# zhengxwen/HIBAG

Measured on AMD Instinct MI355X. Metric: hlaPredict() samples/sec, 10k samples x 100-classifier HLA-B, higher is better.
Workload: dtype f64

## Files before the change

hibag_amd/csrc/hibag_device.h:

```cpp
#ifndef HIBAG_DEVICE_H_
#define HIBAG_DEVICE_H_

#include <stdint.h>
#include <hip/hip_vector_types.h>

#define HIBAG_WAVE 64
#define HIBAG_TAB_N 257
#ifndef HIBAG_TILE
#define HIBAG_TILE 15
#endif
#ifndef HIBAG_CHUNK
#define HIBAG_CHUNK 4
#endif
#ifndef HIBAG_BLOCK_WAVES
#define HIBAG_BLOCK_WAVES 4
#endif
#ifndef HIBAG_ACCUM_WAVES
#define HIBAG_ACCUM_WAVES 4
#endif
#define HIBAG_TILE_META (4 + HIBAG_TILE)
static_assert(HIBAG_TILE <= 16, "cell rows are packed 4 bits each");
#define HIBAG_MAX_NWP 12

#define HIBAG_CHUNK_DWORDS(nwp) (HIBAG_CHUNK * ((nwp) + 2))
#define HIBAG_PLIST_DWORDS 32
#define HIBAG_PLIST_END 0x80000000u
#define HIBAG_PLIST_STORE 0x40000000u
#ifndef HIBAG_STORED_PER_VISIT
#define HIBAG_STORED_PER_VISIT 7
#endif
#define HIBAG_ENGINE_VALU 0
#define HIBAG_ENGINE_FP4 1
#define HIBAG_ENGINE_I8 2
#define HIBAG_ENGINE_I8S 3
#define HIBAG_FP4_STEP_SNPS 28
#define HIBAG_FP4_MAX_STEPS 4
#define HIBAG_FP4_STEPS(k) (((k) + HIBAG_FP4_STEP_SNPS - 1) / HIBAG_FP4_STEP_SNPS)
#define HIBAG_FP4_MAX_SNPS 30
#define HIBAG_ENGINE_OF(k, fp4) ((fp4) && (k) <= HIBAG_FP4_MAX_SNPS ? HIBAG_ENGINE_FP4 : (k) < 32 ? HIBAG_ENGINE_I8 : (k) == 32 ? HIBAG_ENGINE_I8S : \
	(fp4) && (k) <= HIBAG_FP4_STEP_SNPS * HIBAG_FP4_MAX_STEPS ? HIBAG_ENGINE_FP4 : HIBAG_ENGINE_VALU)
#define HIBAG_ENGINE_STEPS(e, k) ((e) == HIBAG_ENGINE_FP4 ? (k) <= HIBAG_FP4_MAX_SNPS ? 1 : HIBAG_FP4_STEPS(k) : 1)
#define HIBAG_ENGINE_ROWS(e, k) ((e) == HIBAG_ENGINE_FP4 ? 2 * HIBAG_ENGINE_STEPS(e, k) : ((e) == HIBAG_ENGINE_VALU ? 0 : 4))
#define HIBAG_ENGINE_HAP_DWORDS(e) 12
#define HIBAG_FP4_ENTRY_DWORDS(steps) (8 + 4 * ((steps) - 1))
#define HIBAG_FP4_SCALE_A 54
#define HIBAG_FP4_SCALE_B_LO 54
#define HIBAG_FP4_SCALE_B_HI 55

struct HibagModelView {
	int n_hla;
	int n_classifier;
	int n_snp;
	int n_cell;
	int mask_rows;
	int n_tile;

	const int *n_snp_c;
	const int *nwp;
	const int *snp_off;
	const int *snp_index;
	const int *snp_weight;
	const int *mask_row;
	const int *c_order;
	const int *tile_p0;
	const int *tile_n;
	const uint32_t *tile_meta;
	const uint32_t *cls_cnt;
	const uint32_t *cls_cell;
	const int *cls_off;
	const int *cls_n;
	int n_item, n_split;
	int all_fp4;
	const int *item;
	int n_item_whole, n_item_split;
	const int *item_whole, *item_split;
	double split_heavy_ns, split_rest_ns;
	const int *split_row;
	const int *split_cls;
	const uint64_t *stream_off;
	const uint32_t *stream;
	const double *tab;

	const int *engine;
	const int *n_step;
	int n_valu;
	int n_wide;
	const int *wide_cls;
	int n_wide_scan;
	const int *wide_scan;
	int n_wide_seg;
	const int *wide_seg;
	const uint64_t *wide_seg_off;
	const int *bt_row;
	const uint32_t *hap;
	const uint32_t *hap_off;
	uint32_t hap_dwords;
	const uint64_t *blk_off;
	const int *cls_nblk;
	const uint32_t *plist;
	uint64_t plist_dwords;
	const double *pfac;
	const uint32_t *phdr;
	const uint4 *parow;
	uint64_t parow_blocks;
	int p1_prebuilt;
	const uint32_t *ctile;

	int store_cells;
	const int *cell_row;
	const uint32_t *blk_close;
// ... 37 lines not shown
```

hibag_amd/csrc/hibag_k_pass2.h:

```cpp
#ifndef HIBAG_K_PASS2_H_
#define HIBAG_K_PASS2_H_

typedef uint32_t u32x8 __attribute__((ext_vector_type(8)));

#ifndef ACCUM_OCC
#define ACCUM_OCC 5
#endif

struct AccumAhead {
	u32x8 hv;
	FactorGroup<ACCUM_G>::type F;
	f64x2 winv;
};

__global__ __launch_bounds__(ACCUM_WAVES * HIBAG_WAVE, ACCUM_OCC) void k_accum(HibagModelView M, HibagBatchView B, int n_whole, int K)
{
	__shared__ double tab_s[ACCUM_TAB_N];
	__shared__ double acc_s[ACCUM_WAVES][HIBAG_TILE][HIBAG_WAVE];
#ifdef HIBAG_ACCUM_STAMPS
	__shared__ unsigned long long stamp_s[ACCUM_STAMP_N];
	if (threadIdx.x < ACCUM_STAMP_N) stamp_s[threadIdx.x] = 0;
	unsigned long long stamp_t = 0;
#endif

	const int n_group = B.n_pad / HIBAG_WAVE;
	const int n_gq = ((n_group + 7) / 8 + ACCUM_WAVES - 1) / ACCUM_WAVES;
	const int C = M.n_classifier;
	const int n_item_x = n_gq * M.n_tile;
	const int xcd = blockIdx.x & 7, wx = blockIdx.x >> 3;
	const int wave = __builtin_amdgcn_readfirstlane(threadIdx.x >> 6);
	const int lane = threadIdx.x & 63;
	double (*acc)[HIBAG_WAVE] = acc_s[wave];

	int item = wx, cb = 0, ce = C;
	if (wx >= n_whole) {
		const int rest = n_item_x - n_whole, k = (wx - n_whole) / rest;
		item = n_whole + (wx - n_whole) - k * rest;
		const uint32_t *__restrict__ cum = M.etile_cstart + (size_t)(item % M.n_tile) * (C + 1);
		const uint64_t total = cum[C];
		if (k > 0) cb = chunk_bound(cum, C, (total * (uint64_t)k + K - 1) / K);
		if (k < K - 1) ce = chunk_bound(cum, C, (total * (uint64_t)(k + 1) + K - 1) / K);
		if (cb >= ce) return;
	}
	stage_table(M, tab_s, ACCUM_TAB_N);
	const int jq = item / M.n_tile, tile = item - jq * M.n_tile;
	const int group = (jq * ACCUM_WAVES + wave) * 8 + xcd;
	unsigned long long *flag = B.sync + (size_t)xcd * n_item_x + item;
	if (cb > 0) handover_wait(flag, B, (uint32_t)cb);
#ifdef HIBAG_ACCUM_STAMPS
	int bb_diag = 0, be_diag = 0;
#endif
	if (group < n_group) {
	const int s = group * HIBAG_WAVE + lane;
	const int ncell = M.tile_n[tile];
	const int p0 = M.tile_p0[tile];

	if (cb > 0) {
		double v[HIBAG_TILE];
#pragma unroll
		for (int j = 0; j < HIBAG_TILE; j++) v[j] = load_parked(&B.part[(size_t)(p0 + (j < ncell ? j : 0)) * B.n_pad + s]);
#pragma unroll
		for (int j = 0; j < HIBAG_TILE; j++) acc[j][lane] = v[j];
	} else {
#pragma unroll
		for (int j = 0; j < HIBAG_TILE; j++) acc[j][lane] = 0;
	}

	const ConstPtr<uint32_t> cst = as_const(M.etile_cstart) + (size_t)tile * (C + 1);
	const int bb = __builtin_amdgcn_readfirstlane((int)cst[cb]), be = __builtin_amdgcn_readfirstlane((int)cst[ce]);
#ifdef HIBAG_ACCUM_STAMPS
	if (wave == 0) { bb_diag = bb; be_diag = be; }
#endif
	if (bb < be && !(ABL2_NOLOOP && B.n_pad >= 0)) {
		const uint64_t blk0 = as_const(M.etile_blk0)[tile] + (uint64_t)bb;
		auto bytes32 = [](size_t n) { return n > 0xFFFFFFF0ull ? (int)0xFFFFFFF0u : (int)(uint32_t)n; };
		auto rsrc_flags = [] { int f = 0x00020000; asm volatile("" : "+s"(f)); return f; };
		const __amdgpu_buffer_rsrc_t pr = __builtin_amdgcn_make_buffer_rsrc((void *)(M.parow + blk0 * 64), 0,
			bytes32((size_t)(M.parow_blocks - blk0) * 1024u), rsrc_flags());
		ConstPtr<double> fac = as_const(M.pfac) + blk0 * HIBAG_PLIST_DWORDS;
		ConstPtr<u32x8> eh = (ConstPtr<u32x8>)(as_const(M.ehdr) + blk0 * 8);
		typedef FactorGroup<ACCUM_G>::type AFG;
		const size_t g_bytes = (size_t)group * HIBAG_WAVE * 16u;
		const __amdgpu_buffer_rsrc_t r_bt = __builtin_amdgcn_make_buffer_rsrc((void *)((const char *)B.bt + g_bytes), 0,
			bytes32((size_t)B.bt_rows * B.n_pad * 16u - g_bytes), rsrc_flags());
		const __amdgpu_buffer_rsrc_t r_wi = __builtin_amdgcn_make_buffer_rsrc((void *)((const char *)B.winv + g_bytes), 0,
			bytes32((size_t)C * B.n_pad * 16u - g_bytes), rsrc_flags());
		const __amdgpu_buffer_rsrc_t r_sv = __builtin_amdgcn_make_buffer_rsrc(
			(void *)(B.cells + (size_t)group * (size_t)as_const(M.cell_row)[C] * HIBAG_WAVE), 0,
			bytes32((size_t)as_const(M.cell_row)[C] * HIBAG_WAVE * 8u), rsrc_flags());
		const int vo_a = lane * 16, vo_row = vo_a, vo_sv = lane * 8;
		const uint32_t row_stride = (uint32_t)B.n_pad * 16u;
		constexpr int NS = HIBAG_STORED_PER_VISIT;

		v4i arow, t0, t1;
		double sv[NS];
		double cell = 0;
		auto request_sv = [&](uint32_t w1) {
			const int ns = abl2_stored(w1);
			if (ns > 0) {
				const int sr = (int)(abl2_stored_row(w1) * (uint32_t)(HIBAG_WAVE * 8));
				int vo = vo_sv;
				asm volatile("" : "+v"(vo));
#pragma unroll
				for (int i = 0; i < NS; i++) {
					if (i >= ns) break;
#ifdef HIBAG_ABL2_SVNOLOAD
					asm volatile("" : "=v"(sv[i]));
#elif defined(HIBAG_ABL2_SVX4)
					sv[i] = __builtin_bit_cast(f64x2, __builtin_amdgcn_raw_buffer_load_b128(r_sv, vo + i * HIBAG_WAVE * 8, sr, 2))[0];
#elif defined(HIBAG_ABL2_SVHALF)
					if (i & 1) asm volatile("" : "=v"(sv[i]));
					else sv[i] = __builtin_bit_cast(double, __builtin_amdgcn_raw_buffer_load_b64(r_sv, vo + i * HIBAG_WAVE * 8, sr, 2));
#else
#ifdef HIBAG_SV_PLAIN
					sv[i] = __builtin_bit_cast(double, __builtin_amdgcn_raw_buffer_load_b64(r_sv, vo + i * HIBAG_WAVE * 8, sr, 0));
#else
					sv[i] = __builtin_bit_cast(double, __builtin_amdgcn_raw_buffer_load_b64(r_sv, vo + i * HIBAG_WAVE * 8, sr, 2));
#endif
#endif
				}
			}
		};
		auto request_lane = [&](uint32_t w0, uint32_t w1, int soff_a, f64x2 &winv) {
			arow = __builtin_bit_cast(v4i, __builtin_amdgcn_raw_buffer_load_b128(pr, vo_a, soff_a, 0));
			const int sb = (int)((w0 >> 16) * row_stride);
			t0 = __builtin_bit_cast(v4i, __builtin_amdgcn_raw_buffer_load_b128(r_bt, vo_row, sb, 0));
			t1 = __builtin_bit_cast(v4i, __builtin_amdgcn_raw_buffer_load_b128(r_bt, vo_row, sb + (int)row_stride, 0));
			if (ABL2_NOWINV) winv = f64x2{1.0 + (double)w0, 2.0};
			else winv = __builtin_bit_cast(f64x2, __builtin_amdgcn_raw_buffer_load_b128(r_wi, vo_row, (int)((w0 & 0xFFFFu) * row_stride), 0));
			request_sv(w1);
		};
		auto one_block = [&](const int rel, AccumAhead &cur, AccumAhead &nxt) {
#if defined(HIBAG_ACCUM_PRIO) && HIBAG_ACCUM_PRIO == 1
			__builtin_amdgcn_s_setprio(1);
#elif defined(HIBAG_ACCUM_PRIO) && HIBAG_ACCUM_PRIO == 2
			__builtin_amdgcn_s_setprio(0);
#endif
			const double w_c = cur.winv[0];
			const bool active = w_c > 0;
			const int any = __builtin_popcountll(__ballot(active));
			const double inv_e = cur.winv[1];
			const uint32_t endmask = cur.hv[0];
			const uint32_t gword = cur.hv[6];
			auto live4 = [&](int g) { return g == 0 || gword >= ((uint32_t)(g + 1) << 28); };
			__builtin_amdgcn_sched_barrier(0);
			nxt.hv = eh[rel + 1];
			nxt.F = *(ConstPtr<AFG>)(fac + (size_t)(rel + 1) * HIBAG_PLIST_DWORDS);
			typedef const volatile __attribute__((address_space(4))) uint32_t *TouchPtr;
			const TouchPtr touch = (TouchPtr)(uintptr_t)(fac + (size_t)(rel + 1) * HIBAG_PLIST_DWORDS);
			const uint32_t tch0 = touch[16], tch1 = touch[32], tch2 = touch[48];
			ACCUM_STAMP(0);
			int eval = ABL2_NOEVAL ? 0 : (any != 0 ? (int)(gword >> 28) : 0), eval_b = eval;
			asm volatile("" : "+s"(eval), "+s"(eval_b));
			{
				const int ns = abl2_stored(cur.hv[1]);
				if (!any) asm volatile("v_mov_b64 %0, 0" : "+v"(cell));
				else {
					asm volatile("");
					if (ns > 0) {
						uint32_t jps = cur.hv[6];
#pragma unroll
						for (int i = 0; i < NS; i++) {
							if (i >= ns) break;
#ifdef HIBAG_ABL2_SVNOADD
							asm volatile("" :: "v"(sv[i]));
#else
							__hip_atomic_fetch_add(&acc[(int)(jps & 15)][lane], (sv[i] * inv_e) * w_c, __ATOMIC_RELAXED, __HIP_MEMORY_SCOPE_WORKGROUP);
#endif
							jps >>= 4;
						}
					}
				}
			}
			__builtin_amdgcn_sched_barrier(0);
			ACCUM_STAMP(1);
			v16i D0, D1;
			if (eval) {
				v16f d0, d1;
#pragma unroll
				for (int r = 0; r < 16; r++) { d0[r] = 0.0f; d1[r] = 0.0f; }
				const v8i a8 = {arow[0], arow[1], arow[2], arow[3], 0, 0, 0, 0};
				const v8i b0 = {t0[0], t0[1], t0[2], t0[3], 0, 0, 0, 0};
				const v8i b1 = {t1[0], t1[1], t1[2], t1[3], 0, 0, 0, 0};
				const int sbs = lane >= 32 ? HIBAG_FP4_SCALE_B_HI : HIBAG_FP4_SCALE_B_LO;
				d0 = __builtin_amdgcn_mfma_scale_f32_32x32x64_f8f6f4(a8, b0, d0, 4, 4, 0, HIBAG_FP4_SCALE_A, 0, sbs);
				d1 = __builtin_amdgcn_mfma_scale_f32_32x32x64_f8f6f4(a8, b1, d1, 4, 4, 0, HIBAG_FP4_SCALE_A, 0, sbs);
				D0 = __builtin_bit_cast(v16i, d0);
				D1 = __builtin_bit_cast(v16i, d1);
			}
			__builtin_amdgcn_sched_barrier(0);
			ACCUM_STAMP(2);
			request_lane(cur.hv[2], cur.hv[3], (rel + 1) * 1024, nxt.winv);
			__builtin_amdgcn_sched_barrier(0);
			ACCUM_STAMP(3);
#if defined(HIBAG_ACCUM_PRIO) && HIBAG_ACCUM_PRIO == 1
			__builtin_amdgcn_s_setprio(0);
#elif defined(HIBAG_ACCUM_PRIO) && HIBAG_ACCUM_PRIO == 2
			__builtin_amdgcn_s_setprio(1);
#endif
			if (eval_b) {
				block_own_sample(D0, D1, [&](int g) { return live4(2 * g); });
#ifdef HIBAG_ACCUM_STAMPS
				asm volatile("" :: "v"(D0[0]), "v"(D1[0]));
				ACCUM_STAMP(4);
#endif
				const uint32_t jp_lo = cur.hv[4], jp_hi = cur.hv[5];
				auto fin = [&](double c, bool, int slot) {
					uint32_t row;
					asm volatile("s_bfe_u32 %0, %1, %2" : "=s"(row) : "s"(slot < 16 ? jp_lo : jp_hi), "n"(4 * ((slot >> 1) & 7) | (4 << 16)) : "scc");
					const double v = (c * inv_e) * w_c;
#ifdef HIBAG_ABL2_NOADD
					asm volatile("" :: "v"(v), "s"(row));
#else
					__hip_atomic_fetch_add(&acc[(int)row][lane], v, __ATOMIC_RELAXED, __HIP_MEMORY_SCOPE_WORKGROUP);
#endif
				};
				uint32_t fresh = (cur.hv[1] >> 29) & 1u;
				block_accumulate<ACCUM_G, ACCUM_AHEAD>(fac + (size_t)rel * HIBAG_PLIST_DWORDS, cur.F, endmask, 0u, live4, D0, D1, cell, fresh, tab_s, fin);
			}
			asm volatile("" :: "s"(tch0), "s"(tch1), "s"(tch2), "s"(nxt.hv[7]));
			ACCUM_STAMP(5);
		};

		AccumAhead A, Bn;
		A.hv = eh[0];
		A.F = *(ConstPtr<AFG>)fac;
		request_lane(A.hv[7], A.hv[1], 0, A.winv);
#ifdef HIBAG_ACCUM_STAMPS
		stamp_t = __builtin_readcyclecounter();
#endif
		const int nb = be - bb;
		for (int rel = 0;;) {
			one_block(rel, A, Bn);
			if (++rel >= nb) break;
			one_block(rel, Bn, A);
			if (++rel >= nb) break;
		}
	}

	if (ce < C) for (int j = 0; j < ncell; j++) store_parked(&B.part[(size_t)(p0 + j) * B.n_pad + s], acc[j][lane]);
	else for (int j = 0; j < ncell; j++) B.part[(size_t)(p0 + j) * B.n_pad + s] = acc[j][lane];
	if (tile == 0 && ce == C) ensemble_scalars<8>(M, B, s, nullptr);
	}
#ifdef HIBAG_ACCUM_STAMPS
	__syncthreads();
	if (threadIdx.x < ACCUM_STAMP_N)
		atomicAdd(reinterpret_cast<unsigned long long *>(B.err_dev + 4) + 2000 + threadIdx.x, stamp_s[threadIdx.x]);
	if (threadIdx.x == ACCUM_STAMP_N) atomicAdd(reinterpret_cast<unsigned long long *>(B.err_dev + 4) + 2000 + ACCUM_STAMP_N, (unsigned long long)(be_diag - bb_diag) * ACCUM_WAVES);
#endif
	if (ce < C) handover_post(flag, B.epoch, (uint32_t)ce, B.drop_post == 2 && blockIdx.x == 8 * n_whole);
}

#define CELLS_WAVES 4
#ifndef CELLS_OCC
#define CELLS_OCC 4
#endif
__global__ __launch_bounds__(CELLS_WAVES * HIBAG_WAVE, CELLS_OCC) void k_accum_cells(HibagModelView M, HibagBatchView B)
{
	constexpr int CELLS_V = (HIBAG_TILE + 3) / 4 * 4;
	__shared__ double acc_s[CELLS_WAVES][HIBAG_TILE][HIBAG_WAVE];
	const int n_group = B.n_pad / HIBAG_WAVE;
	const int tq = (M.n_tile + CELLS_WAVES - 1) / CELLS_WAVES;
	const int xcd = blockIdx.x & 7, jb = blockIdx.x >> 3;
	const int wave = __builtin_amdgcn_readfirstlane(threadIdx.x >> 6);
	const int lane = threadIdx.x & 63;
	const int group = (jb / tq) * 8 + xcd, tile = (jb % tq) * CELLS_WAVES + wave;
	if (group >= n_group || tile >= M.n_tile) return;
	const int s = group * HIBAG_WAVE + lane;
	const int C = M.n_classifier;
	const int ncell = M.tile_n[tile];
	double (*acc)[HIBAG_WAVE] = acc_s[wave];
#pragma unroll
	for (int q = 0; q < HIBAG_TILE; q++) acc[q][lane] = 0;

	typedef uint32_t u32x8 __attribute__((ext_vector_type(8)));
	const ConstPtr<u32x8> ct = as_const(reinterpret_cast<const u32x8 *>(M.ctile)) + tile;
	const double *__restrict__ const group_rows = B.cells + (size_t)group * (size_t)as_const(M.cell_row)[C] * HIBAG_WAVE + lane;
	struct Visit { u32x8 rec; double w, inv; };
	auto visit = [&](int c) {
		Visit x;
		x.rec = ct[(size_t)c * M.n_tile];
		x.w = B.cw[(size_t)c * B.n_pad + s];
		x.inv = B.inv[(size_t)c * B.n_pad + s];
		return x;
	};
	auto fetch = [&](const Visit &x, double (&v)[CELLS_V]) {
		const int n = (int)((x.rec[0] >> 8) & 31u);
		const double *__restrict__ rows = group_rows + (size_t)(x.rec[5] & 0x7FFFFFFu) * HIBAG_WAVE;
#pragma unroll
		for (int g = 0; g < HIBAG_TILE; g += 4) {
			if (g >= n) break;
#pragma unroll
			for (int i = g; i < g + 4; i++) v[i] = __builtin_nontemporal_load(rows + (size_t)(i < n ? i : n - 1) * HIBAG_WAVE);
		}
	};
	auto add = [&](int c, const Visit &x, const double (&v)[CELLS_V]) {
		const bool active = x.w > 0;
		if (__ballot(active) == 0) return;
// ... 37 lines not shown
```

hibag_amd/csrc/hibag_model.hip:

```cpp

#include "hibag_internal.h"

namespace hibag_detail {



void build_table(double *tab)
{
	const double min_rare_freq = 1e-5;
	for (int i = 0; i < HIBAG_TAB_N; i++) tab[i] = std::exp(i * std::log(min_rare_freq));
	tab[0] = 1;
	for (int i = 0; i < HIBAG_TAB_N; i++)
		if (!std::isfinite(tab[i])) tab[i] = 0;
}

int check_classifier_args(hibag_hip_model *m, int n_snp_c, const int32_t *snpidx, int n_haplo,
	const double *freq, const int32_t *hla)
{
	if (!m) return hibag_fail(HIBAG_HIP_EINVAL, "model is NULL");
	if (m->finalized) return hibag_fail(HIBAG_HIP_ESTATE, "model already finalized");
	if (n_snp_c < 0 || n_snp_c > HIBAG_HIP_MAX_SNP_IN_CLASSIFIER)
		return hibag_fail(HIBAG_HIP_EINVAL, "there are too many SNP markers in a classifier (%d > %d).",
			n_snp_c, HIBAG_HIP_MAX_SNP_IN_CLASSIFIER);
	if (n_haplo < 0 || (n_haplo > 0 && (!freq || !hla)))
// ... 369 lines not shown
			}
			me[0] = (uint32_t)k;
			me[2] = (uint32_t)jpack; me[3] = (uint32_t)(jpack >> 32);
			{
				uint64_t jp = 0;
				int nl = 0, ns = 0;
				for (int j = 0; j < tile_n[t]; j++)
					if (cell_chunks[c][tile_p0[t] + j] && !stored_big(c, tile_p0[t] + j)) {
						jp |= (uint64_t)j << (4 * nl++);
						if (store_mode != 1) m->second_pass_pairs += pass2_evaluates(c) ? cell_pairs[c][tile_p0[t] + j] : 0;
					}
				for (int j = 0; j < tile_n[t]; j++)
					if (stored_big(c, tile_p0[t] + j)) jp |= (uint64_t)j << (4 * (nl + ns++));
				tile_jpack[(size_t)c * n_tile + t] = jp;
				tile_nlist[(size_t)c * n_tile + t] = (uint32_t)nl;
				tile_nstored[(size_t)c * n_tile + t] = (uint32_t)ns;
				if (store_mode == 2) tile_k0[(size_t)c * n_tile + t] = (uint32_t)n_stored_c[c];
				n_stored_c[c] += ns;
			}
			k_first += k;
			for (int j = 0; j < tile_n[t]; j++)
				if (!cell_chunks[c][tile_p0[t] + j]) me[4 + k++] = (uint32_t)j << 24;
		}
	}
	if (cls_cnt.empty()) { cls_cnt.push_back(0); cls_cell.push_back(0); }

	std::vector<int> item, item_whole, split_row(std::max(C, 1), -1), split_cls, wide_cls;
	double split_heavy_ns = 0, split_rest_ns = 0;
	{
		std::vector<double> work(C, 0.0);
		double typical = 0;
		int n_typ = 0;
		for (int c = 0; c < C; c++) {
			work[c] = (double)pairs[c] * (mfma_nkb[c] ? 50.0 * (0.5 + 0.5 * n_step[c]) : 48.0 * nwp[c]);
			if (mfma_nkb[c]) { typical += work[c]; n_typ++; }
			split_rest_ns += work[c];
		}
		typical = n_typ ? typical / n_typ : 0;
		std::vector<std::pair<double, std::vector<int>>> items, whole;
		for (int c = 0; c < C; c++) {
			if (n_step[c] > 1) { wide_cls.push_back(c); continue; }
			whole.push_back({work[c], {c, 0, cls_n[c], 0}});
			int nseg = 1;
			if (!mfma_nkb[c] && typical > 0 && work[c] > 3 * typical)
				nseg = (int)std::min<double>(64, std::max(2.0, std::floor(work[c] / typical)));
			if (nseg == 1 || cls_n[c] < 2) {
				items.push_back({work[c], {c, 0, cls_n[c], 0}});
				continue;
			}
			split_heavy_ns = std::max(split_heavy_ns, (double)pairs[c] * 18.0 * nwp[c]);
			split_row[c] = 1;
			split_cls.push_back(c);
			uint64_t total = 0, acc = 0, chunk0 = 0;
			for (int i = 0; i < cls_n[c]; i++) total += cls_cnt[cls_off[c] + i] + 1;
			int i0 = 0, k = 1;
			for (int i = 0; i < cls_n[c]; i++) {
				acc += cls_cnt[cls_off[c] + i] + 1;
				const bool last = i + 1 == cls_n[c];
				if (last || acc * nseg >= total * k) {
					uint64_t chunks = 0;
					for (int j = i0; j <= i; j++) chunks += cls_cnt[cls_off[c] + j];
					items.push_back({work[c] * (double)(chunks + 1) / (double)total, {c, i0, i + 1, (int)chunk0}});
					chunk0 += chunks;
					i0 = i + 1;
					while (k < nseg && acc * nseg >= total * k) k++;
				}
			}
		}
		std::stable_sort(whole.begin(), whole.end(), [](const auto &a, const auto &b) { return a.first > b.first; });
		for (const auto &it : whole) item_whole.insert(item_whole.end(), it.second.begin(), it.second.end());
		std::stable_sort(items.begin(), items.end(), [](const auto &a, const auto &b) { return a.first > b.first; });
		for (const auto &it : items) item.insert(item.end(), it.second.begin(), it.second.end());
	}

	std::vector<uint32_t> plist;
	struct SlotRange { size_t first, n; int c; };
	std::vector<SlotRange> slot_ranges;
	std::vector<uint64_t> blk_off(std::max(C, 1), 0), seg_off((size_t)std::max(C, 1) * n_tile, 0);
	std::vector<uint32_t> seg_nblk((size_t)std::max(C, 1) * n_tile, 0);
	long long dbg_b1 = 0, dbg_b2 = 0, dbg_seg = 0;
	std::vector<int> cell_row((size_t)C + 1, 0);
	for (int c = 0; c < C; c++)
		cell_row[c + 1] = cell_row[c] + (store_mode == 1 || split_row[c] >= 0 ? cls_n[c] : store_mode == 2 ? n_stored_c[c] : 0);
	std::vector<uint32_t> ehdr, etile_cstart((size_t)n_tile * (C + 1), 0);
	std::vector<uint64_t> etile_blk0(std::max(n_tile, 1), 0);
	hap.insert(hap.end(), HIBAG_ENGINE_HAP_DWORDS(HIBAG_ENGINE_FP4), 0u);
	while (hap.size() % 4) hap.push_back(0u);
	for (int t = 0; t < n_tile && store_mode != 1; t++) {
		etile_blk0[t] = plist.size() / HIBAG_PLIST_DWORDS;
		for (int c = 0; c < C; c++) {
			const size_t ct = (size_t)c * n_tile + t;
			etile_cstart[(size_t)t * (C + 1) + c] = (uint32_t)(plist.size() / HIBAG_PLIST_DWORDS - etile_blk0[t]);
			const size_t first = plist.size();
			int nb = 0;
			if (pass2_evaluates(c) && tile_nlist[ct] > 0)
				nb = append_pair_blocks(starts[c].data(), nh, tile_h1[t], tile_h2[t], tile_p0[t], tile_n[t],
					(uint32_t)m->cls[c].freq.size(), plist, nullptr, store_mode == 2 ? stored[c].data() : nullptr);
			if (nb > 0) slot_ranges.push_back({first, plist.size() - first, c});
			const int ns = (int)tile_nstored[ct];
			const int nvb = std::max(nb, (ns + HIBAG_STORED_PER_VISIT - 1) / HIBAG_STORED_PER_VISIT);
			for (int b = nb; b < nvb; b++) plist.insert(plist.end(), HIBAG_PLIST_DWORDS, 0u);
			dbg_b2 += nvb; dbg_seg += nvb > 0;
			uint64_t jp = tile_jpack[ct];
			uint64_t jps = jp >> (4 * tile_nlist[ct]);
			uint32_t srow = (uint32_t)cell_row[c] + tile_k0[ct];
			for (int b = 0; b < nvb; b++) {
				uint64_t jq = 0;
				if (b < nb)
					for (int i = 0; i < HIBAG_PLIST_DWORDS; i++)
						if (plist[first + (size_t)b * HIBAG_PLIST_DWORDS + i] >> 31) {
							if (!(i & 1)) return hibag_fail(HIBAG_HIP_ESTATE, "internal: a cell of classifier %d closes at an even slot", c);
							jq |= (jp & 15u) << (4 * (i >> 1));
							jp >>= 4;
						}
				const int nsb = std::max(0, std::min(HIBAG_STORED_PER_VISIT, ns - HIBAG_STORED_PER_VISIT * b));
				if (c > 0xFFFF) return hibag_fail(HIBAG_HIP_EINVAL, "too many classifiers (%d) for the second pass's block headers", C);
				const uint32_t bt = (uint32_t)(HIBAG_ENGINE_ROWS(engine[c], n_snp_c[c]) > 0 ? bt_row[c] : 0);
				if (bt > 0xFFFFu) return hibag_fail(HIBAG_HIP_EINVAL, "too many classifiers for the matrix engine's operand rows");
				const uint32_t h[8] = {
					(uint32_t)c | (bt << 16), srow | ((uint32_t)nsb << 25),
					0u, 0u,
					(uint32_t)jq, (uint32_t)(jq >> 32),
					(uint32_t)jps, 0u};
				ehdr.insert(ehdr.end(), h, h + 8);
				jps >>= 4 * nsb;
				srow += (uint32_t)nsb;
			}
		}
		etile_cstart[(size_t)t * (C + 1) + C] = (uint32_t)(plist.size() / HIBAG_PLIST_DWORDS - etile_blk0[t]);
	}
	const uint64_t estream_blocks = plist.size() / HIBAG_PLIST_DWORDS + 4;
	plist.insert(plist.end(), 4 * HIBAG_PLIST_DWORDS, 0u);
	ehdr.resize(estream_blocks * 8, 0u);
	for (uint64_t b = 0; b + 1 < estream_blocks; b++) { ehdr[b * 8 + 2] = ehdr[(b + 1) * 8]; ehdr[b * 8 + 3] = ehdr[(b + 1) * 8 + 1]; }
	const uint64_t p1_base = plist.size();
	std::vector<uint32_t> blk_close;
	std::vector<int> wseg, wide_scan;
	std::vector<uint64_t> wseg_off;
	for (int c = 0; c < C; c++) {
		if (!mfma_nkb[c]) continue;
		blk_off[c] = plist.size();
		if (n_step[c] > 1) {
			const bool whole = (int)wide_cls.size() >= 8;
			const long long seg_pairs = whole ? (1ll << 62) : std::max<long long>(512, 6000 / n_step[c]);
			bool any_seg = false;
			int p_lo = 0, h1_lo = 0, h2_lo = 0, row = 0, h1 = 0, h2 = 0;
			long long acc_pairs = 0;
			int rows_in_seg = 0;
			for (int p = 0; p < P; p++) {
				acc_pairs += cell_pairs[c][p];
				rows_in_seg += cell_pairs[c][p] != 0;
				int nh1 = h1, nh2 = h2 + 1;
				if (nh2 == nh) { nh1++; nh2 = nh1; }
				if (acc_pairs >= seg_pairs || p + 1 == P) {
					const size_t off = plist.size();
					const int nb = append_pair_blocks(starts[c].data(), nh, h1_lo, h2_lo, p_lo, p + 1 - p_lo, (uint32_t)m->cls[c].freq.size(),
						plist, stored[c].data(), nullptr);
					if (nb > 0) { wseg.insert(wseg.end(), {c, row, nb, whole ? 1 : 0}); wseg_off.push_back(off); any_seg = true; }
					row += rows_in_seg; rows_in_seg = 0; acc_pairs = 0;
					p_lo = p + 1; h1_lo = nh1; h2_lo = nh2;
				}
				h1 = nh1; h2 = nh2;
			}
			if (!whole || !any_seg) wide_scan.push_back(c);
			cls_nblk[c] = (int)((plist.size() - blk_off[c]) / HIBAG_PLIST_DWORDS);
			slot_ranges.push_back({(size_t)blk_off[c], plist.size() - (size_t)blk_off[c], c});
			dbg_b1 += cls_nblk[c];
			for (int b = 0; b < cls_nblk[c] && store_mode; b++) blk_close.push_back(0);
			continue;
		}
		cls_nblk[c] = append_pair_blocks(starts[c].data(), nh, 0, 0, 0, P, (uint32_t)m->cls[c].freq.size(), plist,
			store_mode ? stored[c].data() : nullptr, nullptr);
		slot_ranges.push_back({(size_t)blk_off[c], plist.size() - (size_t)blk_off[c], c});
		dbg_b1 += cls_nblk[c];
		uint32_t closed = 0;
		for (int b = 0; b < cls_nblk[c] && store_mode; b++) {
			blk_close.push_back(closed);
			for (int i = 0; i < HIBAG_PLIST_DWORDS; i++) closed += (plist[blk_off[c] + (size_t)b * HIBAG_PLIST_DWORDS + i] >> 30) & 1u;
		}
	}
	if (blk_close.empty()) blk_close.push_back(0);
	(void)valu_pairs;
	if (getenv("HIBAG_DEBUG_MODEL"))
		fprintf(stderr, "[hibag model] %d classifiers, %d tiles, pairs %lld; blocks of 32: pass 1 %lld, pass 2 %lld in %lld (classifier, tile) segments; "
			"pair lists %.1f MB + factors %.1f MB + block headers %.1f MB, haplotype table %.1f KB, VALU-engine stream %.1f MB\n",
			C, n_tile, (long long)m->pair_evals, dbg_b1, dbg_b2, dbg_seg, plist.size() * 4e-6, plist.size() * 8e-6, plist.size() / 32 * 16e-6,
			hap.size() * 4e-3, stream.size() * 4e-6);
	plist.insert(plist.end(), 4 * HIBAG_PLIST_DWORDS, 0u);
	std::vector<double> pfac(plist.size(), 0.0);
	for (const SlotRange &r : slot_ranges) {
		const std::vector<double> &freq = m->cls[r.c].freq;
		const uint32_t H = (uint32_t)freq.size();
		auto ff_of = [&](uint32_t e) { return e < H ? 2 * freq[e] : e == H ? 0.0 : freq[e - H - 1]; };
		auto f_of = [&](uint32_t e) { return e < H ? freq[e] : e == H ? 0.0 : freq[e - H - 1]; };
		for (size_t i = r.first; i < r.first + r.n; i++) pfac[i] = ff_of(plist[i] & 0xFFFFu) * f_of((plist[i] >> 16) & 0x3FFFu);
	}
	std::vector<uint32_t> phdr(plist.size() / HIBAG_PLIST_DWORDS * 4, 0u);
	for (size_t b = 0; b < plist.size() / HIBAG_PLIST_DWORDS; b++) {
		uint32_t ends = 0, stores = 0, live = 0;
		for (int i = 0; i < HIBAG_PLIST_DWORDS; i++) {
			const uint32_t w = plist[b * HIBAG_PLIST_DWORDS + i];
			if (w & HIBAG_PLIST_END) ends |= 1u << i;
			if (w >= (HIBAG_PLIST_END | HIBAG_PLIST_STORE)) stores |= 1u << i;
			if (pfac[b * HIBAG_PLIST_DWORDS + i] != 0.0) live |= 1u << i;
		}
		live |= ends;
		int n_valid = 0;
		while (n_valid < 32 && (live >> n_valid)) n_valid++;
		phdr[4 * b] = ends; phdr[4 * b + 1] = stores; phdr[4 * b + 2] = (uint32_t)n_valid;
	}
	uint32_t closed_before = 0;
	for (uint64_t b = 0; b < estream_blocks; b++) {
		const uint32_t groups = (phdr[4 * b + 2] + 3) / 4;
		ehdr[b * 8 + 7] = ehdr[b * 8];
		ehdr[b * 8] = phdr[4 * b];
		ehdr[b * 8 + 1] |= closed_before << 29;
		ehdr[b * 8 + 6] = (ehdr[b * 8 + 6] & 0x0FFFFFFFu) | (groups << 28);
		if (groups > 0) closed_before = (phdr[4 * b] >> (4 * groups - 1)) & 1u;
	}
	for (uint64_t b = 0; b + 1 < estream_blocks; b++) ehdr[b * 8 + 3] = ehdr[(b + 1) * 8 + 1];
	const size_t n_blocks_all = plist.size() / HIBAG_PLIST_DWORDS;
	double pre_mb = 128;
	if (const char *e = getenv("HIBAG_PREBUILT_MB")) pre_mb = atof(e);
	bool p1_prebuilt = false;
	{
		size_t fp4_p1_blocks = 0;
		for (int c = 0; c < C; c++) if (pass2_evaluates(c)) fp4_p1_blocks += (size_t)cls_nblk[c];
		p1_prebuilt = fp4_p1_blocks > 0 && (double)(n_blocks_all) * 1024.0 <= pre_mb * 1e6;
	}
	const size_t parow_blocks = p1_prebuilt ? n_blocks_all : (size_t)estream_blocks;
	std::vector<uint32_t> parow(parow_blocks * 256, 0u);
	for (const SlotRange &r : slot_ranges) {
		if (!pass2_evaluates(r.c)) continue;
		const uint32_t *tab_c = hap.data() + hap_off[r.c];
		for (size_t i = r.first; i < r.first + r.n; i++) {
			const size_t b = i / HIBAG_PLIST_DWORDS, sl = i % HIBAG_PLIST_DWORDS;
			if (b >= parow_blocks) break;
			const uint32_t *e1 = tab_c + (size_t)(plist[i] & 0xFFFFu) * 12, *e2 = tab_c + (size_t)((plist[i] >> 16) & 0x3FFFu) * 12;
			for (int h = 0; h < 2; h++)
				for (int d = 0; d < 4; d++) parow[(b * 64 + (size_t)h * 32 + sl) * 4 + d] = e1[4 * h + d] + e2[4 * h + d];
		}
	}
	std::vector<uint32_t> ctile((size_t)std::max(C, 1) * n_tile * 8 + 8, 0);
	for (int c = 0; c < C; c++)
		for (int t = 0; t < n_tile; t++) {
			uint32_t *r = &ctile[((size_t)c * n_tile + t) * 8];
			const uint32_t *me = &tile_meta[((size_t)c * n_tile + t) * HIBAG_TILE_META];
			const uint64_t off = seg_off[(size_t)c * n_tile + t];
			if (bt_row[c] > 0xFFFF) return hibag_fail(HIBAG_HIP_EINVAL, "too many classifiers for the matrix engine's operand rows");
			(void)me;
			const int k_last = n_snp_c[c] - HIBAG_FP4_STEP_SNPS * (n_step[c] - 1);
			r[0] = (uint32_t)mfma_nkb[c] | ((uint32_t)k_last << 2 & 0xFCu) | (tile_nlist[(size_t)c * n_tile + t] << 8) |
			       ((uint32_t)(n_step[c] - 1) << 13) | ((uint32_t)bt_row[c] << 16);
			r[1] = hap_off[c];
			r[2] = (uint32_t)off; r[3] = (uint32_t)(off >> 32);
			r[4] = seg_nblk[(size_t)c * n_tile + t];
			const uint64_t row = (uint64_t)cell_row[c] + tile_k0[(size_t)c * n_tile + t];
			if (row >> 27) return hibag_fail(HIBAG_HIP_EINVAL, "the model has too many allele pairs to store their sums");
			r[5] = (uint32_t)row | (tile_nstored[(size_t)c * n_tile + t] << 27);
			r[6] = (uint32_t)tile_jpack[(size_t)c * n_tile + t]; r[7] = (uint32_t)(tile_jpack[(size_t)c * n_tile + t] >> 32);
		}

	std::vector<int> arena;
	auto put = [&](const std::vector<int> &v) {
		size_t off = arena.size();
		arena.insert(arena.end(), v.begin(), v.end());
		if (v.empty()) arena.push_back(0);
		return off;
	};
// ... 291 lines not shown
```

Baseline: 8.101 million.

## Pack two classifiers' partial pair blocks into one mixed second-pass block

When a classifier's second-pass pair list leaves its last 32-slot block partly empty, the host builder now fills the remaining slots with the next classifier's pairs and flags the header as mixed. The header records the classifier offset, the operand-row offset and the split slot. The accumulate kernel loads the second classifier's B operands and weights for mixed blocks and issues two extra masked MFMAs. It then switches the weight and inverse at the split slot, so fewer padded blocks are processed. In exchange, mixed blocks cost extra loads and MFMAs, add register pressure and branching in the hot loop, and the packing is on by default unless an environment variable disables it.

Result: no change. 8.100 million, median of 6 (-0.0%).

```diff
diff --git a/hibag_amd/csrc/hibag_device.h b/hibag_amd/csrc/hibag_device.h
--- a/hibag_amd/csrc/hibag_device.h
+++ b/hibag_amd/csrc/hibag_device.h
@@ -26,6 +26,7 @@
 #define HIBAG_PLIST_DWORDS 32
 #define HIBAG_PLIST_END 0x80000000u
 #define HIBAG_PLIST_STORE 0x40000000u
+#define HIBAG_EHDR_MIXED 0x40000000u
 #ifndef HIBAG_STORED_PER_VISIT
 #define HIBAG_STORED_PER_VISIT 7
 #endif
diff --git a/hibag_amd/csrc/hibag_k_pass2.h b/hibag_amd/csrc/hibag_k_pass2.h
--- a/hibag_amd/csrc/hibag_k_pass2.h
+++ b/hibag_amd/csrc/hibag_k_pass2.h
@@ -95,9 +95,16 @@
 		v4i arow, t0, t1;
 		double sv[NS];
 		double cell = 0;
-		auto request_sv = [&](uint32_t w1) {
+		auto request_sv = [&](uint32_t w0, uint32_t w1) {
 			const int ns = abl2_stored(w1);
-			if (ns > 0) {
+			if (w1 & HIBAG_EHDR_MIXED) {
+				const uint32_t c2 = (w0 & 0xFFFFu) + (w1 & 0xFFu), r2 = (w0 >> 16) + ((w1 >> 8) & 0xFFu);
+				const int sb = (int)(r2 * row_stride);
+				const f64x2 u0 = __builtin_bit_cast(f64x2, __builtin_amdgcn_raw_buffer_load_b128(r_bt, vo_row, sb, 0));
+				const f64x2 u1 = __builtin_bit_cast(f64x2, __builtin_amdgcn_raw_buffer_load_b128(r_bt, vo_row, sb + (int)row_stride, 0));
+				const f64x2 u2 = __builtin_bit_cast(f64x2, __builtin_amdgcn_raw_buffer_load_b128(r_wi, vo_row, (int)(c2 * row_stride), 0));
+				sv[0] = u0[0]; sv[1] = u0[1]; sv[2] = u1[0]; sv[3] = u1[1]; sv[4] = u2[0]; sv[5] = u2[1];
+			} else if (ns > 0) {
 				const int sr = (int)(abl2_stored_row(w1) * (uint32_t)(HIBAG_WAVE * 8));
 				int vo = vo_sv;
 				asm volatile("" : "+v"(vo));
@@ -128,7 +135,7 @@
 			t1 = __builtin_bit_cast(v4i, __builtin_amdgcn_raw_buffer_load_b128(r_bt, vo_row, sb + (int)row_stride, 0));
 			if (ABL2_NOWINV) winv = f64x2{1.0 + (double)w0, 2.0};
 			else winv = __builtin_bit_cast(f64x2, __builtin_amdgcn_raw_buffer_load_b128(r_wi, vo_row, (int)((w0 & 0xFFFFu) * row_stride), 0));
-			request_sv(w1);
+			request_sv(w0, w1);
 		};
 		auto one_block = [&](const int rel, AccumAhead &cur, AccumAhead &nxt) {
 #if defined(HIBAG_ACCUM_PRIO) && HIBAG_ACCUM_PRIO == 1
@@ -138,7 +145,13 @@
 #endif
 			const double w_c = cur.winv[0];
 			const bool active = w_c > 0;
-			const int any = __builtin_popcountll(__ballot(active));
+			const uint32_t w1c = cur.hv[1];
+			const bool mixed = (w1c & HIBAG_EHDR_MIXED) != 0;
+			const int split = mixed ? (int)((w1c >> 16) & 31u) : 0;
+			const double w_2 = sv[4], inv_2 = sv[5];
+			const int any1 = __builtin_popcountll(__ballot(active));
+			const int any2 = mixed ? __builtin_popcountll(__ballot(w_2 > 0)) : 0;
+			const int any = any1 + any2;
 			const double inv_e = cur.winv[1];
 			const uint32_t endmask = cur.hv[0];
 			const uint32_t gword = cur.hv[6];
@@ -179,12 +192,26 @@
 				v16f d0, d1;
 #pragma unroll
 				for (int r = 0; r < 16; r++) { d0[r] = 0.0f; d1[r] = 0.0f; }
-				const v8i a8 = {arow[0], arow[1], arow[2], arow[3], 0, 0, 0, 0};
 				const v8i b0 = {t0[0], t0[1], t0[2], t0[3], 0, 0, 0, 0};
 				const v8i b1 = {t1[0], t1[1], t1[2], t1[3], 0, 0, 0, 0};
 				const int sbs = lane >= 32 ? HIBAG_FP4_SCALE_B_HI : HIBAG_FP4_SCALE_B_LO;
-				d0 = __builtin_amdgcn_mfma_scale_f32_32x32x64_f8f6f4(a8, b0, d0, 4, 4, 0, HIBAG_FP4_SCALE_A, 0, sbs);
-				d1 = __builtin_amdgcn_mfma_scale_f32_32x32x64_f8f6f4(a8, b1, d1, 4, 4, 0, HIBAG_FP4_SCALE_A, 0, sbs);
+				if (mixed) {
+					const bool lo = (lane & 31) < split;
+					const bool k_lo = lo && any1 != 0, k_hi = !lo && any2 != 0;
+					const v8i a_lo = {k_lo ? arow[0] : 0, k_lo ? arow[1] : 0, k_lo ? arow[2] : 0, k_lo ? arow[3] : 0, 0, 0, 0, 0};
+					const v8i a_hi = {k_hi ? arow[0] : 0, k_hi ? arow[1] : 0, k_hi ? arow[2] : 0, k_hi ? arow[3] : 0, 0, 0, 0, 0};
+					const v4i u0 = __builtin_bit_cast(v4i, f64x2{sv[0], sv[1]}), u1 = __builtin_bit_cast(v4i, f64x2{sv[2], sv[3]});
+					const v8i c0 = {u0[0], u0[1], u0[2], u0[3], 0, 0, 0, 0};
+					const v8i c1 = {u1[0], u1[1], u1[2], u1[3], 0, 0, 0, 0};
+					d0 = __builtin_amdgcn_mfma_scale_f32_32x32x64_f8f6f4(a_lo, b0, d0, 4, 4, 0, HIBAG_FP4_SCALE_A, 0, sbs);
+					d1 = __builtin_amdgcn_mfma_scale_f32_32x32x64_f8f6f4(a_lo, b1, d1, 4, 4, 0, HIBAG_FP4_SCALE_A, 0, sbs);
+					d0 = __builtin_amdgcn_mfma_scale_f32_32x32x64_f8f6f4(a_hi, c0, d0, 4, 4, 0, HIBAG_FP4_SCALE_A, 0, sbs);
+					d1 = __builtin_amdgcn_mfma_scale_f32_32x32x64_f8f6f4(a_hi, c1, d1, 4, 4, 0, HIBAG_FP4_SCALE_A, 0, sbs);
+				} else {
+					const v8i a8 = {arow[0], arow[1], arow[2], arow[3], 0, 0, 0, 0};
+					d0 = __builtin_amdgcn_mfma_scale_f32_32x32x64_f8f6f4(a8, b0, d0, 4, 4, 0, HIBAG_FP4_SCALE_A, 0, sbs);
+					d1 = __builtin_amdgcn_mfma_scale_f32_32x32x64_f8f6f4(a8, b1, d1, 4, 4, 0, HIBAG_FP4_SCALE_A, 0, sbs);
+				}
 				D0 = __builtin_bit_cast(v16i, d0);
 				D1 = __builtin_bit_cast(v16i, d1);
 			}
@@ -205,15 +232,21 @@
 				ACCUM_STAMP(4);
 #endif
 				const uint32_t jp_lo = cur.hv[4], jp_hi = cur.hv[5];
+				double wv = w_c, iv = inv_e, wv2 = w_2, iv2 = inv_2;
+				if (mixed) {
+					if (!any1) { wv = 0; iv = 0; }
+					if (!any2) { wv2 = 0; iv2 = 0; }
+				}
 				auto fin = [&](double c, bool, int slot) {
 					uint32_t row;
 					asm volatile("s_bfe_u32 %0, %1, %2" : "=s"(row) : "s"(slot < 16 ? jp_lo : jp_hi), "n"(4 * ((slot >> 1) & 7) | (4 << 16)) : "scc");
-					const double v = (c * inv_e) * w_c;
+					const double v = (c * iv) * wv;
 #ifdef HIBAG_ABL2_NOADD
 					asm volatile("" :: "v"(v), "s"(row));
 #else
 					__hip_atomic_fetch_add(&acc[(int)row][lane], v, __ATOMIC_RELAXED, __HIP_MEMORY_SCOPE_WORKGROUP);
 #endif
+					if (slot + 1 == split) { wv = wv2; iv = iv2; asm volatile("" : "+v"(wv), "+v"(iv)); }
 				};
 				uint32_t fresh = (cur.hv[1] >> 29) & 1u;
 				block_accumulate<ACCUM_G, ACCUM_AHEAD>(fac + (size_t)rel * HIBAG_PLIST_DWORDS, cur.F, endmask, 0u, live4, D0, D1, cell, fresh, tab_s, fin);
diff --git a/hibag_amd/csrc/hibag_model.hip b/hibag_amd/csrc/hibag_model.hip
--- a/hibag_amd/csrc/hibag_model.hip
+++ b/hibag_amd/csrc/hibag_model.hip
@@ -475,50 +475,90 @@
 	std::vector<int> cell_row((size_t)C + 1, 0);
 	for (int c = 0; c < C; c++)
 		cell_row[c + 1] = cell_row[c] + (store_mode == 1 || split_row[c] >= 0 ? cls_n[c] : store_mode == 2 ? n_stored_c[c] : 0);
+	bool pack = true;
+	if (const char *e = getenv("HIBAG_PASS2_PACK")) pack = atoi(e) != 0;
 	std::vector<uint32_t> ehdr, etile_cstart((size_t)n_tile * (C + 1), 0);
 	std::vector<uint64_t> etile_blk0(std::max(n_tile, 1), 0);
+	long long dbg_mixed = 0, dbg_pairs2 = 0;
 	hap.insert(hap.end(), HIBAG_ENGINE_HAP_DWORDS(HIBAG_ENGINE_FP4), 0u);
 	while (hap.size() % 4) hap.push_back(0u);
+	std::vector<uint32_t> vis;
 	for (int t = 0; t < n_tile && store_mode != 1; t++) {
 		etile_blk0[t] = plist.size() / HIBAG_PLIST_DWORDS;
+		size_t open_at = 0, open_h = 0;
+		int open_fill = 0, open_c = -1;
+		uint32_t open_bt = 0;
 		for (int c = 0; c < C; c++) {
 			const size_t ct = (size_t)c * n_tile + t;
 			etile_cstart[(size_t)t * (C + 1) + c] = (uint32_t)(plist.size() / HIBAG_PLIST_DWORDS - etile_blk0[t]);
-			const size_t first = plist.size();
-			int nb = 0;
+			const uint32_t pad_idx = (uint32_t)m->cls[c].freq.size() * 0x10001u;
+			vis.clear();
 			if (pass2_evaluates(c) && tile_nlist[ct] > 0)
-				nb = append_pair_blocks(starts[c].data(), nh, tile_h1[t], tile_h2[t], tile_p0[t], tile_n[t],
-					(uint32_t)m->cls[c].freq.size(), plist, nullptr, store_mode == 2 ? stored[c].data() : nullptr);
-			if (nb > 0) slot_ranges.push_back({first, plist.size() - first, c});
+				append_pair_blocks(starts[c].data(), nh, tile_h1[t], tile_h2[t], tile_p0[t], tile_n[t],
+					(uint32_t)m->cls[c].freq.size(), vis, nullptr, store_mode == 2 ? stored[c].data() : nullptr);
+			size_t nsl = vis.size();
+			while (nsl > 0 && !(vis[nsl - 1] & HIBAG_PLIST_END)) nsl--;
+			for (size_t i = 0; i < nsl; i++) dbg_pairs2 += (vis[i] & ~(HIBAG_PLIST_END | HIBAG_PLIST_STORE)) != pad_idx;
 			const int ns = (int)tile_nstored[ct];
-			const int nvb = std::max(nb, (ns + HIBAG_STORED_PER_VISIT - 1) / HIBAG_STORED_PER_VISIT);
-			for (int b = nb; b < nvb; b++) plist.insert(plist.end(), HIBAG_PLIST_DWORDS, 0u);
-			dbg_b2 += nvb; dbg_seg += nvb > 0;
+			if (nsl == 0 && ns == 0) continue;
+			if (c > 0xFFFF) return hibag_fail(HIBAG_HIP_EINVAL, "too many classifiers (%d) for the second pass's block headers", C);
+			const uint32_t bt = (uint32_t)(HIBAG_ENGINE_ROWS(engine[c], n_snp_c[c]) > 0 ? bt_row[c] : 0);
+			if (bt > 0xFFFFu) return hibag_fail(HIBAG_HIP_EINVAL, "too many classifiers for the matrix engine's operand rows");
 			uint64_t jp = tile_jpack[ct];
 			uint64_t jps = jp >> (4 * tile_nlist[ct]);
+			auto rows_of = [&](size_t i0, size_t i1, int s0, uint64_t &jq) {
+				for (size_t i = i0; i < i1; i++)
+					if (vis[i] & HIBAG_PLIST_END) {
+						const int slot = s0 + (int)(i - i0);
+						if (!(slot & 1)) return false;
+						jq |= (jp & 15u) << (4 * (slot >> 1));
+						jp >>= 4;
+					}
+				return true;
+			};
+			size_t i0 = 0;
+			if (ns > 0) open_c = -1;
+			else if (open_c >= 0 && pack && nsl > 0 && c - open_c <= 0xFF && bt >= open_bt && bt - open_bt <= 0xFFu) {
+				size_t k = 0;
+				for (size_t i = 0; i < nsl && (int)i < HIBAG_PLIST_DWORDS - open_fill; i++)
+					if (vis[i] & HIBAG_PLIST_END) k = i + 1;
+				if (k > 0) {
+					std::copy(vis.begin(), vis.begin() + (long)k, plist.begin() + (long)(open_at + open_fill));
+					slot_ranges.push_back({open_at + open_fill, k, c});
+					uint64_t jq = (uint64_t)ehdr[open_h + 4] | (uint64_t)ehdr[open_h + 5] << 32;
+					if (!rows_of(0, k, open_fill, jq)) return hibag_fail(HIBAG_HIP_ESTATE, "internal: a cell of classifier %d closes at an even slot", c);
+					ehdr[open_h + 4] = (uint32_t)jq; ehdr[open_h + 5] = (uint32_t)(jq >> 32);
+					ehdr[open_h + 1] = (uint32_t)(c - open_c) | (bt - open_bt) << 8 | (uint32_t)open_fill << 16 | HIBAG_EHDR_MIXED;
+					dbg_mixed++;
+					i0 = k;
+				}
+				open_c = -1;
+			}
+			const int nb = (int)((nsl - i0 + HIBAG_PLIST_DWORDS - 1) / HIBAG_PLIST_DWORDS);
+			const int nvb = std::max(nb, (ns + HIBAG_STORED_PER_VISIT - 1) / HIBAG_STORED_PER_VISIT);
+			if (nsl > i0) slot_ranges.push_back({plist.size(), nsl - i0, c});
 			uint32_t srow = (uint32_t)cell_row[c] + tile_k0[ct];
 			for (int b = 0; b < nvb; b++) {
+				const size_t at = plist.size();
+				const size_t s0 = i0 + (size_t)b * HIBAG_PLIST_DWORDS, s1 = b < nb ? std::min(nsl, s0 + HIBAG_PLIST_DWORDS) : s0;
+				plist.insert(plist.end(), HIBAG_PLIST_DWORDS, b < nb ? pad_idx : 0u);
+				if (b < nb) std::copy(vis.begin() + (long)s0, vis.begin() + (long)s1, plist.begin() + (long)at);
 				uint64_t jq = 0;
-				if (b < nb)
-					for (int i = 0; i < HIBAG_PLIST_DWORDS; i++)
-						if (plist[first + (size_t)b * HIBAG_PLIST_DWORDS + i] >> 31) {
-							if (!(i & 1)) return hibag_fail(HIBAG_HIP_ESTATE, "internal: a cell of classifier %d closes at an even slot", c);
-							jq |= (jp & 15u) << (4 * (i >> 1));
-							jp >>= 4;
-						}
+				if (!rows_of(s0, s1, 0, jq)) return hibag_fail(HIBAG_HIP_ESTATE, "internal: a cell of classifier %d closes at an even slot", c);
 				const int nsb = std::max(0, std::min(HIBAG_STORED_PER_VISIT, ns - HIBAG_STORED_PER_VISIT * b));
-				if (c > 0xFFFF) return hibag_fail(HIBAG_HIP_EINVAL, "too many classifiers (%d) for the second pass's block headers", C);
-				const uint32_t bt = (uint32_t)(HIBAG_ENGINE_ROWS(engine[c], n_snp_c[c]) > 0 ? bt_row[c] : 0);
-				if (bt > 0xFFFFu) return hibag_fail(HIBAG_HIP_EINVAL, "too many classifiers for the matrix engine's operand rows");
 				const uint32_t h[8] = {
 					(uint32_t)c | (bt << 16), srow | ((uint32_t)nsb << 25),
 					0u, 0u,
 					(uint32_t)jq, (uint32_t)(jq >> 32),
 					(uint32_t)jps, 0u};
+				open_h = ehdr.size();
 				ehdr.insert(ehdr.end(), h, h + 8);
 				jps >>= 4 * nsb;
 				srow += (uint32_t)nsb;
-			}
+				open_c = b == nb - 1 && nvb == nb && nsb == 0 && s1 - s0 < HIBAG_PLIST_DWORDS ? c : -1;
+				open_at = at; open_fill = (int)(s1 - s0); open_bt = bt;
+			}
+			dbg_b2 += nvb; dbg_seg++;
 		}
 		etile_cstart[(size_t)t * (C + 1) + C] = (uint32_t)(plist.size() / HIBAG_PLIST_DWORDS - etile_blk0[t]);
 	}
@@ -575,9 +615,11 @@
 	if (blk_close.empty()) blk_close.push_back(0);
 	(void)valu_pairs;
 	if (getenv("HIBAG_DEBUG_MODEL"))
-		fprintf(stderr, "[hibag model] %d classifiers, %d tiles, pairs %lld; blocks of 32: pass 1 %lld, pass 2 %lld in %lld (classifier, tile) segments; "
+		fprintf(stderr, "[hibag model] %d classifiers, %d tiles, pairs %lld; blocks of 32: pass 1 %lld, pass 2 %lld in %lld (classifier, tile) segments "
+			"(%s: %lld mixed, %.1f evaluated pairs per block); "
 			"pair lists %.1f MB + factors %.1f MB + block headers %.1f MB, haplotype table %.1f KB, VALU-engine stream %.1f MB\n",
-			C, n_tile, (long long)m->pair_evals, dbg_b1, dbg_b2, dbg_seg, plist.size() * 4e-6, plist.size() * 8e-6, plist.size() / 32 * 16e-6,
+			C, n_tile, (long long)m->pair_evals, dbg_b1, dbg_b2, dbg_seg, pack ? "packed" : "unpacked", dbg_mixed,
+			dbg_b2 ? (double)dbg_pairs2 / (double)dbg_b2 : 0.0, plist.size() * 4e-6, plist.size() * 8e-6, plist.size() / 32 * 16e-6,
 			hap.size() * 4e-3, stream.size() * 4e-6);
 	plist.insert(plist.end(), 4 * HIBAG_PLIST_DWORDS, 0u);
 	std::vector<double> pfac(plist.size(), 0.0);
```
